# alevar/tiebrush

Hardware: AMD Instinct MI355X
Metric: input alignment records/sec collapsed (tiebrush) + bases/sec covered (tiecov) (higher is better)
Workload: dtype int64; 1 GPU; c3: 64 synthetic sorted BAMs x 5000000 100bp reads per GPU, --clip collapse + tiecov -c -j of the result; records_per_gpu=320000000, groups_out=25086541, parallelism=files-per-rank x1, ranks_seen=1, resident=SoA in HBM before the timed region, contexts=3

## Files before the change

### tiebrush_amd/csrc/tbk_api.hip

```cpp
#include <sys/mman.h>

#include <algorithm>
#include <chrono>
#include <mutex>
#include <vector>
#include <new>

#include "tbk_internal.h"

namespace {
std::mutex g_reg_m;
struct RegEntry {
  void* p;
  int users;
};
std::vector<RegEntry> g_reg;
}

static void release_registered(tbk_ctx* ctx) {
  if (ctx->registered.empty()) return;
  (void)hipStreamSynchronize(ctx->stream);
  const auto r0 = std::chrono::steady_clock::now();
  struct RP {
    tbk_ctx* c;
// ... 369 lines not shown
  return ctx->aux;
}

tbk_ctx* tbk_side_ctx(tbk_ctx* ctx) {
  if (!ctx->side_ctx && tbk_create(ctx->device, &ctx->side_ctx) != 0) ctx->side_ctx = nullptr;
  if (ctx->side_ctx) {
    ctx->side_ctx->profiling = ctx->profiling;
    ctx->side_ctx->dbg = ctx->dbg;
  }
  return ctx->side_ctx;
}
int tbk_side_begin(tbk_ctx* side, size_t arena_hint) {
  if (hipSetDevice(side->device) != hipSuccess) return TBK_EHIP;
  tbk_prof_begin_call(side);
  return ws_begin_call(side, arena_hint);
}
void tbk_side_end(tbk_ctx* side) { tbk_prof_end_call(side); }

static void merge_side_times(tbk_ctx* ctx) {
  if (!ctx->side_times_pending || !ctx->side_ctx) return;
  ctx->side_times_pending = false;
  for (auto& t : ctx->side_ctx->last_times) {
    bool found = false;
    for (auto& u : ctx->last_times)
      if (strcmp(u.name, t.name) == 0) {
        u.ms += t.ms;
        u.launches += t.launches;
        found = true;
        break;
      }
    if (!found) ctx->last_times.push_back(t);
  }
}

static int yd_stage_on(tbk_ctx* run_on, void* job, size_t hint) {
  if (hipSetDevice(run_on->device) != hipSuccess) return TBK_EHIP;
  tbk_prof_begin_call(run_on);
  int rc = ws_begin_call(run_on, hint);
  if (rc == 0) rc = tbk_collapse_yd_run(run_on, job);
  tbk_prof_end_call(run_on);
  return rc;
}

static int finish_yd(tbk_ctx* ctx) {
  if (!ctx->yd_pending) return 0;
  ctx->yd_worker->wait();
  ctx->yd_pending = false;
  ctx->ws_base_off = 0;
  if (ctx->yd_ctx) {
    ctx->last_times = ctx->yd_ctx->last_times;
    if (ctx->yd_rc != 0) ctx->last_error = ctx->yd_ctx->last_error;
  }
  return ctx->yd_rc;
}

void tbk_debug_parse(const char* spec, TbkDebug* out) {
  *out = TbkDebug();
  if (!spec) return;
  std::string s(spec);
  size_t at = 0;
  while (at < s.size()) {
    size_t end = s.find(',', at);
    if (end == std::string::npos) end = s.size();
    const std::string kv = s.substr(at, end - at);
    at = end + 1;
    const size_t eq = kv.find('=');
    const std::string k = kv.substr(0, eq), v = eq == std::string::npos ? std::string("1") : kv.substr(eq + 1);
    const unsigned long long u = strtoull(v.c_str(), nullptr, 0);
    const bool on = v != "0";
    if (k == "path") out->path = v == "sort" ? 1 : (v == "window" ? 2 : 0);
    else if (k == "raw") out->raw = on ? 1 : 0;
    else if (k == "sort") out->sort = v == "radix" ? 1 : (v == "runs" ? 2 : 0);
    else if (k == "scan") out->scan = v == "lookback" ? 1 : (v == "3pass" ? 2 : 0);
    else if (k == "hash_mask") out->hash_mask = (uint32_t)u;
    else if (k == "qhash_mask") out->qhash_mask = u;
    else if (k == "yd_wave_min") out->yd_wave_min = (uint32_t)u;
    else if (k == "yd_bgrid") out->yd_bgrid = (uint32_t)u;
    else if (k == "yd_radix") out->yd_radix = on;
    else if (k == "yd_literal") out->yd_literal = on;
    else if (k == "yd_front") out->yd_front_split = v == "split";
    else if (k == "yd_own_arena") out->yd_own_arena = on;
    else if (k == "wg_stats") out->wg_stats = on;
    else if (k == "wg_og") out->wg_og = (uint32_t)u;
    else if (k == "wg_dense_verify") out->wg_dense_verify = on;
    else if (k == "wg_rank_merge") out->wg_rank_merge = on;
    else if (k == "wg_back") out->wg_back_split = v == "split";
    else if (k == "cov_legacy") out->cov_legacy = on;
    else if (k == "cov_bundle_scan") out->cov_bundle_scan = on;
    else if (k == "cov_prep") out->cov_prep = on;
    else if (k == "cov_tile_cap") out->cov_tile_cap = u;
    else if (k == "junc_radix") out->junc_radix = on;
    else if (k == "no_junc_agg") out->no_junc_agg = on;
    else if (k == "jh_cap") out->jh_cap = (uint32_t)u;
    else if (k == "index_chain") out->index_chain = on;
    else if (k == "no_register") out->no_register = on;
    else if (k == "phases") out->phases = on;
    else if (k == "no_bounce") out->no_bounce = on;
    else if (k == "fmt_slice") out->fmt_slice = u;
  }
}

extern "C" {

int tbk_abi_version(void) { return TBK_ABI_VERSION; }

int tbk_set_debug(tbk_ctx* ctx, const char* spec) {
  if (!ctx) return TBK_EINVAL;
  tbk_debug_parse(spec, &ctx->dbg);
  if (ctx->yd_ctx) ctx->yd_ctx->dbg = ctx->dbg;
  if (ctx->side_ctx) ctx->side_ctx->dbg = ctx->dbg;
  return 0;
}

const char* tbk_strerror(int s) {
  switch (s) {
    case TBK_OK: return "ok";
    case TBK_EINVAL: return "invalid argument";
    case TBK_ENOMEM: return "out of memory";
    case TBK_EHIP: return "HIP runtime error";
    case TBK_E2BIG: return "output capacity too small";
    case TBK_EUNSUPPORTED: return "option or input outside the supported/pinned semantics";
    case TBK_EUNSORTED: return "input not coordinate-sorted";
    case TBK_EFATALOP: return "unknown opcode (tiecov accepts only M/I/D/N/S)";
    case TBK_ECOLLISION: return "key hash collision survived all reseeds";
    case TBK_ENODEVICE: return "no usable gfx950 device";
  }
  return "unknown status";
}

int tbk_create(int device_ordinal, tbk_ctx** out) {
  if (!out) return TBK_EINVAL;
  *out = nullptr;
  int ndev = 0;
  if (hipGetDeviceCount(&ndev) != hipSuccess || ndev <= 0 || device_ordinal < 0 || device_ordinal >= ndev) return TBK_ENODEVICE;
  tbk_ctx* ctx = new (std::nothrow) tbk_ctx();
  if (!ctx) return TBK_ENOMEM;
  ctx->device = device_ordinal;
  tbk_debug_parse(getenv("TBK_DEBUG"), &ctx->dbg);
  bool ok = hipSetDevice(device_ordinal) == hipSuccess;
  hipDeviceProp_t prop;
  if (ok && hipGetDeviceProperties(&prop, device_ordinal) == hipSuccess) ctx->num_cu = prop.multiProcessorCount;
  ok = ok && hipStreamCreateWithFlags(&ctx->own_stream, hipStreamNonBlocking) == hipSuccess;
  ctx->stream = ctx->own_stream;
  ok = ok && hipMalloc((void**)&ctx->d_scalars, 64 * sizeof(uint64_t)) == hipSuccess;
  if (ok) ctx->d_err = (uint32_t*)(ctx->d_scalars + 15);
  ok = ok && hipHostMalloc((void**)&ctx->h_scalars, (64 + 4096) * sizeof(uint64_t), hipHostMallocDefault) == hipSuccess;
  if (!ok) {
    tbk_destroy(ctx);
    return TBK_EHIP;
  }
  *out = ctx;
  return 0;
}

int tbk_collapse_finish_yd(tbk_ctx* ctx) {
  if (!ctx) return TBK_EINVAL;
  return finish_yd(ctx);
}

void tbk_destroy(tbk_ctx* ctx) {
  if (!ctx) return;
  (void)finish_yd(ctx);
  tbk_bam_release(ctx);
  delete ctx->yd_worker;
  ctx->yd_worker = nullptr;
  delete ctx->side_worker;
// ... 449 lines not shown
```

### tiebrush_amd/csrc/tbk_internal.h

```cpp
#pragma once
#include <hip/hip_runtime.h>
#include <stdint.h>
#include <stdio.h>
#include <string.h>

#include <string>
#include <condition_variable>
#include <functional>
#include <mutex>
#include <thread>
#include <utility>
#include <vector>

#include "../../include/tbk.h"

enum : uint32_t {
  TBK_DERR_UNSORTED = 1u << 0,
  TBK_DERR_COLLISION = 1u << 1,
  TBK_DERR_FATALOP = 1u << 2,
  TBK_DERR_SPAN = 1u << 3,
  TBK_DERR_NCIGAR = 1u << 4,
  TBK_DERR_FRACTIONAL = 1u << 5,
  TBK_DERR_OVERFLOW = 1u << 6,
  TBK_DERR_INTERNAL = 1u << 7,
  TBK_DERR_BIGBUCKET = 1u << 8,
  TBK_DERR_RAWORDER = 1u << 9
};

struct KTime {
  const char* name;
  hipEvent_t a, b;
};

struct TbkWorker {
  std::thread th;
  std::mutex m;
  std::condition_variable cv;
  std::function<void()> job;
  bool busy = false, quit = false, started = false;
  void post(std::function<void()> j) {
    {
      std::lock_guard<std::mutex> lk(m);
      if (!started) {
        started = true;
        th = std::thread([this]() {
          std::unique_lock<std::mutex> lk2(m);
          for (;;) {
            cv.wait(lk2, [&] { return quit || (bool)job; });
            if (quit) return;
            std::function<void()> run = std::move(job);
            job = nullptr;
            lk2.unlock();
            run();
            lk2.lock();
            busy = false;
            cv.notify_all();
          }
        });
      }
      job = std::move(j);
      busy = true;
    }
    cv.notify_all();
  }
  void wait() {
    std::unique_lock<std::mutex> lk(m);
    cv.wait(lk, [&] { return !busy; });
  }
  ~TbkWorker() {
    {
      std::lock_guard<std::mutex> lk(m);
      quit = true;
    }
    cv.notify_all();
    if (th.joinable()) th.join();
  }
};

struct TbkDebug {
  int path = 0;
  int raw = -1;
  int sort = 0;
  int scan = 0;
  uint32_t hash_mask = 0xFFFFFFFFu;
  uint64_t qhash_mask = ~0ull;
  uint32_t yd_wave_min = 0;
  uint32_t yd_bgrid = 0;
  bool yd_radix = false;
  bool yd_literal = false;
  bool yd_front_split = false;
  bool yd_own_arena = false;
  uint32_t wg_og = 0;
  bool wg_stats = false;
  bool wg_dense_verify = false, wg_rank_merge = false;
  bool wg_back_split = false;
  bool cov_legacy = false, cov_bundle_scan = false, cov_prep = false, junc_radix = false, no_junc_agg = false;
  uint64_t cov_tile_cap = 0;
  uint32_t jh_cap = 0;
  bool index_chain = false;
  bool no_register = false;
  bool no_bounce = false;
  bool phases = false;
  uint64_t fmt_slice = 0;
};
void tbk_debug_parse(const char* spec, TbkDebug* out);

struct tbk_ctx {
  int device = 0;
  TbkDebug dbg;
  hipStream_t own_stream = nullptr;
  hipStream_t stream = nullptr;
  hipStream_t aux = nullptr;
  hipEvent_t aux_done = nullptr;
  char* ws = nullptr;
  size_t ws_cap = 0, ws_off = 0;
  size_t ws_top = 0;
  bool ws_top_mode = false;
  bool ws_borrowed = false;
  std::vector<std::pair<char*, size_t>> ws_overflow;
  size_t ws_over_used = 0;
  uint32_t* d_err = nullptr;
  uint64_t* d_scalars = nullptr;
  uint64_t* h_scalars = nullptr;
  hipEvent_t stage_ev = nullptr;
  char* d_view = nullptr;
  size_t d_view_cap = 0;
  struct ViewPrep {
    bool valid = false;
    const void* cig = nullptr;
    uint32_t n = 0;
    int32_t *start = nullptr, *end = nullptr, *yi = nullptr;
    uint32_t *jcnt = nullptr, *ridx = nullptr;
    const void* agg = nullptr;
    uint32_t agg_tiles = 0;
    uint64_t n_bases = 0, sum_abs = 0, n_junc = 0;
    uint32_t err = 0;
  } view_prep;
  bool profiling = false;
  std::vector<KTime> ktimes;
  std::vector<hipEvent_t> ev_pool;
  size_t ev_used = 0;
  std::vector<tbk_kernel_time> last_times;
  std::string last_error;
  tbk_collapse_route route{};
  int num_cu = 256;
  void* yd_job = nullptr;
  tbk_ctx* yd_ctx = nullptr;
  TbkWorker* yd_worker = nullptr;
  bool yd_pending = false;
  int yd_rc = 0;
  size_t ws_base_off = 0;
  tbk_ctx* side_ctx = nullptr;
  TbkWorker* side_worker = nullptr;
  bool side_times_pending = false;
  std::vector<void*> registered;
  char* d_unpack = nullptr;
  size_t d_unpack_cap = 0;
  std::vector<uint8_t> unpack_tbm;
  void* bam_dev = nullptr;
  void* enc = nullptr;
  void* ix = nullptr;
  void* stager = nullptr;
  char* bounce = nullptr;
  char* kept = nullptr;
  size_t kept_cap = 0;
  uint32_t kept_n = 0;
  uint32_t* kept_rep = nullptr;
  double* kept_yc = nullptr;
  int64_t* kept_yx = nullptr;
  int32_t* kept_yd = nullptr;
  char* d_names = nullptr;
  uint64_t* d_name_off = nullptr;
  uint32_t n_names = 0;
  void* fmt_pin[2] = {nullptr, nullptr};
  size_t fmt_pin_cap = 0;
// ... 107 lines not shown
```

### tiebrush_amd/csrc/wgroup.h

```cpp
#pragma once
#include <stdlib.h>

#include "strategy.hpp"
#include "tbk_internal.h"

struct WgOut {
  uint32_t ng = 0, np = 0;
  uint64_t *ghi = nullptr, *glo = nullptr;
  uint32_t* gmem = nullptr;
  uint32_t* gpoff = nullptr;
  uint16_t* pfile = nullptr;
  uint32_t* pgrp = nullptr;
  uint64_t* gfmask = nullptr;
  uint32_t* rec_sg = nullptr;
  double* yc = nullptr;
  uint32_t* ns = nullptr;
  long long *yxin = nullptr, *ydin = nullptr;
  unsigned long long* rep = nullptr;
  uint32_t* first = nullptr;
  uint8_t* tie = nullptr;
  uint32_t *gperm = nullptr, *ginv = nullptr;
  bool ties_done = false;
};

struct WgDirectOut {
  uint32_t cap = 0;
  uint32_t* rep = nullptr;
  double* yc = nullptr;
  int64_t* yx = nullptr;
  int32_t *g_start = nullptr, *g_end = nullptr, *rep_effend = nullptr;
  uint64_t* g_key = nullptr;
  int strategy = 0;
};

int tbk_window_groups(tbk_ctx* ctx, const tbkd::ColIn& I, int strategy, const uint64_t* chi, const uint64_t* clo, const uint32_t* cval,
                      const uint32_t* ceff, uint32_t m, const uint32_t* d_run_off, uint64_t* scratch_hi, uint64_t* scratch_lo,
                      bool want_rec_sg, uint64_t seed, WgOut* out, uint32_t* err_bits, const tbkd::ColOpt* raw_opt = nullptr, bool part = false,
                      const WgDirectOut* direct = nullptr );
bool tbk_window_supported(uint32_t k);
inline bool tbk_yd_by_list(const tbk_ctx* ctx, uint32_t k) { return 2u * k <= 128u && !ctx->dbg.yd_radix; }

int tbk_partial_reduce_device(tbk_ctx* ctx, int strategy, const int32_t* rows, uint32_t n2, const uint32_t* run_off_host, uint32_t n_runs,
                              const uint32_t* cig, tbk_groups_out* out, tbk_cov_in* view, const uint32_t* md_off = nullptr,
                              const uint8_t* md = nullptr, const uint8_t* md_has = nullptr);
```

### tiebrush_amd/csrc/wgroup.hip

```cpp
#include <stdlib.h>

#include <algorithm>

#include "dev_common.hpp"
#include "strategy.hpp"
#include "tbk_internal.h"
#include "wgroup.h"

namespace {

constexpr int WG_NT = 512;
constexpr int WG_E = 8;
constexpr int WG_CAP = WG_NT * WG_E;
constexpr uint32_t WG_T = 1024;
constexpr uint32_t WG_KS = 2048;
constexpr int WG_NW = WG_NT / 64;
constexpr int WG_R = 4;
constexpr int WG_RS = 1;
constexpr int WG_RR = 1;

__global__ void wg_sample_k(const uint64_t* __restrict__ chi, uint32_t m, uint32_t s, uint32_t ns, uint64_t* __restrict__ shi) {
  uint32_t j = blockIdx.x * blockDim.x + threadIdx.x;
  if (j >= ns) return;
  uint64_t d = (uint64_t)j * s;
// ... 158 lines not shown
      }
    } else {
      for (uint32_t j = t; j < i1 - i0; j += 256) key[j] = chi[i0 + j] >> 2;
    }
    __syncthreads();
    uint32_t f_first;
    {
      uint32_t lo = 0, hi = k;
      while (hi - lo > 1) {
        const uint32_t mid = (lo + hi) >> 1;
        if (s_run[mid] <= i0)
          lo = mid;
        else
          hi = mid;
      }
      f_first = lo;
    }
    uint32_t seg = 0;
    for (uint32_t f = f_first; f < k; ++f) {
      const uint32_t a = s_run[f], b = s_run[f + 1];
      if (a >= i1) break;
      if (b <= i0 || a == b) continue;
      const uint32_t sa = a > i0 ? a : i0, sb = b < i1 ? b : i1;
      const bool has_lo = sa > a;
      const bool cont = has_lo && c_f == f && c_end == sa;
      const uint64_t klo = !has_lo ? 0ull : cont ? c_klast : (RAW ? raw_key(rtid[sa - 1], rpos[sa - 1]) : (chi[sa - 1] >> 2));
      const uint64_t khi = key[sb - 1 - i0];
      uint32_t r_lo, r_hi;
      bool found = false, have_v = false;
      if (cont && sb == b) {
        r_lo = c_rhi;
        r_hi = nW;
        found = true;
      } else if (cont) {
        r_lo = c_rhi;
        const bool le = r_lo + t < nW && wprobe <= khi;
        const uint64_t mb = __ballot(le);
        uint32_t* sl = s_loc[(g + seg) & 1u];
        if ((t & 63u) == 0) sl[t >> 6] = (uint32_t)__builtin_popcountll(mb);
        __syncthreads();
        const uint32_t c = sl[0] + sl[1] + sl[2] + sl[3];
        if (c < 256u) {
          r_hi = r_lo + c;
          found = true;
          have_v = true;
        }
      }
      ++seg;
      if (!found) {
        upper_bounds2(klo, !has_lo, khi, sb == b, &r_lo, &r_hi);
        r_hi = sb == b ? nW : r_hi;
      }
      const uint64_t v_mine = wprobe;
      if (sb != b) {
        c_f = f;
        c_end = sb;
        c_rhi = r_hi;
        c_klast = khi;
        wprobe = r_hi + t < nW ? W[r_hi + t] : ~0ull;
      } else {
        c_f = ~0u;
      }
      for (uint32_t r = r_lo + t; r < r_hi; r += 256) {
        const uint64_t v = have_v ? v_mine : W[r];
        uint32_t lo = sa - i0, hi = sb - i0;
        while (lo < hi) {
          const uint32_t mid = lo + ((hi - lo) >> 1);
          if (key[mid] < v)
            lo = mid + 1;
          else
            hi = mid;
        }
        offT[(size_t)f * nrows + (r + 1)] = i0 + lo;
      }
      if (RAW) {
        for (uint32_t j = sa + t; j < sb; j += 256) {
          const uint64_t pk = j > sa ? key[j - 1 - i0] : klo;
          bad |= pk > key[j - i0];
        }
      }
    }
  }
  if (RAW && bad) atomicOr(err, TBK_DERR_RAWORDER);
}
__global__ void wg_offsets_edges_k(const uint32_t* __restrict__ run_off, uint32_t k, uint32_t nrows, uint32_t* __restrict__ offT) {
  const uint32_t f = blockIdx.x;
  const uint32_t a = run_off[f], b = run_off[f + 1];
  uint32_t* col = offT + (size_t)f * nrows;
  if (threadIdx.x == 0) {
    col[0] = a;
    col[nrows - 1] = b;
  }
  if (a == b)
    for (uint32_t r = 1 + threadIdx.x; r + 1 < nrows; r += blockDim.x) col[r] = a;
}
__global__ __launch_bounds__(256) void wg_offsets_transpose_k(const uint32_t* __restrict__ offT, uint32_t k, uint32_t nrows, uint32_t* __restrict__ off,
                                                             uint32_t* __restrict__ wbase) {
  __shared__ uint32_t tile[64][65];
  const uint32_t r0 = blockIdx.x * 64, f0 = blockIdx.y * 64;
  const uint32_t tx = threadIdx.x & 63, ty = threadIdx.x >> 6;
  const uint32_t start = (wbase && tx < k) ? offT[(size_t)tx * nrows] : 0u;
  for (uint32_t y = ty; y < 64; y += 4) {
    const uint32_t f = f0 + y, r = r0 + tx;
    if (f < k && r < nrows) tile[y][tx] = offT[(size_t)f * nrows + r];
  }
  __syncthreads();
  for (uint32_t y = ty; y < 64; y += 4) {
    const uint32_t r = r0 + y, f = f0 + tx;
    const bool in = f < k && r < nrows;
    const uint32_t v = in ? tile[tx][y] : 0u;
    if (in) off[(size_t)r * k + f] = v;
    if (wbase) {
      const uint32_t sum = wave_sum(in ? v - start : 0u);
      if (tx == 0 && r < nrows) wbase[r] = sum;
    }
  }
}
struct WgRaw {
  ColIn I;
  ColOpt O;
  unsigned long long* n_pass;
  unsigned long long* n_slots;
  uint32_t all_slots;
  uint32_t sparse;
};
constexpr uint32_t WG_NSPREAD = 64, WG_SPREAD_STRIDE = 16;
__device__ __forceinline__ void wg_count(unsigned long long* base, unsigned long long v) {
  atomicAdd(base + (size_t)(blockIdx.x & (WG_NSPREAD - 1u)) * WG_SPREAD_STRIDE, v);
}
__device__ __forceinline__ uint32_t wave_seg_max(uint32_t x, uint32_t f, uint32_t* fo) {
#define WG_SEG_STEP(ctrl, rm)                                                                  \
  {                                                                                            \
    const uint32_t xo = (uint32_t)__builtin_amdgcn_update_dpp(0, (int)x, ctrl, rm, 0xf, false); \
    const uint32_t fq = (uint32_t)__builtin_amdgcn_update_dpp(0, (int)f, ctrl, rm, 0xf, false); \
    x = f ? x : (xo > x ? xo : x);                                                             \
    f |= fq;                                                                                   \
  }
  WG_SEG_STEP(0x111, 0xf)
  WG_SEG_STEP(0x112, 0xf)
  WG_SEG_STEP(0x114, 0xf)
  WG_SEG_STEP(0x118, 0xf)
  WG_SEG_STEP(0x142, 0xa)
  WG_SEG_STEP(0x143, 0xc)
#undef WG_SEG_STEP
  *fo = f;
  return x;
}
struct RawA {
  int32_t pos, tidv, ppos, ptid;
  uint32_t fl_mq_sc;
  int32_t nh;
  uint32_t c0, nc;
};
struct RawRec {
  uint64_t hi, lo, rk, prk;
  uint32_t x;
  uint32_t err;
  bool pass;
};
__device__ __forceinline__ RawA wg_raw_a(const ColIn& I, uint32_t i, bool need_prev) {
  RawA a;
  a.pos = I.pos[i];
  a.tidv = I.tid[i];
  a.fl_mq_sc = (uint32_t)I.flag[i] | ((uint32_t)I.mapq[i] << 16) | (strand_code(I.strand[i]) << 24);
  a.nh = I.nh[i];
  a.c0 = I.cig_off[i];
// ... 1621 lines not shown
      const uint32_t src = rsrc[e];
      const int4* rp = reinterpret_cast<const int4*>(rows + (size_t)src * TBK_PARTIAL_ROW);
      const int4 a = rp[0], b = rp[1], c = rp[2];
      const uint32_t eff = (uint32_t)a.w;
      if (m == q || eff < beff) {
        beff = eff;
        best = src;
      }
      yc += (double)(uint32_t)b.z;
      yx += (uint32_t)b.w;
      yd = (uint32_t)c.x > yd && c.x > 0 ? (uint32_t)c.x : yd;
      if (hashed && m > q && !strategy_equal(I, strategy, src, rsrc[e0])) atomicOr(err, TBK_DERR_COLLISION);
    }
    T.rep[wb + gid] = best;
    T.yc[wb + gid] = yc;
    if (yx > 0xFFFFFFFFull) atomicOr(err, TBK_DERR_OVERFLOW);
    T.yx[wb + gid] = (uint32_t)yx;
    T.yd[wb + gid] = yd;
    T.khi[wb + gid] = h;
    T.klo[wb + gid] = l;
    ++gid;
  }
  if (t == 0) T.wg_cnt[w] = tot;
}

__global__ __launch_bounds__(256) void pr_compact_k(uint32_t nw, const uint32_t* __restrict__ wbase, PrTemp T, const uint32_t* __restrict__ gbase,
                                                   uint32_t cap, uint32_t* __restrict__ o_rep,
                                                   double* __restrict__ o_yc, int64_t* __restrict__ o_yx, int32_t* __restrict__ o_yd,
                                                   int32_t* __restrict__ o_start, int32_t* __restrict__ o_end, uint64_t* __restrict__ o_key,
                                                   int strategy) {
  const uint32_t w = blockIdx.x * 4u + (threadIdx.x >> 6);
  if (w >= nw) return;
  const uint32_t ng = T.wg_cnt[w];
  if (!ng) return;
  const uint32_t wb = wbase[w], gb = gbase[w];
  for (uint32_t g = threadIdx.x & 63u; g < ng; g += 64) {
    const uint32_t o = gb + g;
    if (o >= cap) continue;
    const uint32_t r = T.rep[wb + g], yxv = T.yx[wb + g], ydv = T.yd[wb + g];
    const double ycv = T.yc[wb + g];
    const uint64_t h = T.khi[wb + g], l = T.klo[wb + g];
    o_rep[o] = r;
    o_yc[o] = ycv;
    o_yx[o] = (int64_t)yxv;
    o_yd[o] = (int32_t)ydv;
    if (o_start || o_end || o_key) {
      const int32_t start = (int32_t)((h >> 2) & 0x7FFFFFFFull);
      if (o_start) o_start[o] = start;
      if (o_end) o_end[o] = start + (int32_t)(uint32_t)(l >> 32) - 1;
      if (o_key) {
        const uint32_t word = (uint32_t)l;
        uint32_t shape = 0;
        if (strategy == TBK_STRAT_CIGAR || strategy == TBK_STRAT_CLIP) {
          if (word == (0x80000000u | C_M)) shape = 0x80000000u;
          if ((word >> 30) == 3u) shape = word;
        }
        o_key[2 * (size_t)o] = h;
        o_key[2 * (size_t)o + 1] = (l & 0xFFFFFFFF00000000ull) | shape;
      }
    }
  }
}

__global__ __launch_bounds__(64) void wg_spread_sum_k(const unsigned long long* __restrict__ spread, unsigned long long* __restrict__ n_pass,
                                                      unsigned long long* __restrict__ n_slots) {
  const unsigned long long a = wave_sum(spread[(size_t)threadIdx.x * WG_SPREAD_STRIDE]);
  const unsigned long long b = wave_sum(spread[(size_t)(WG_NSPREAD + threadIdx.x) * WG_SPREAD_STRIDE]);
  if (threadIdx.x == 0) {
    *n_pass += a;
    *n_slots += b;
  }
}

}

bool tbk_window_supported(uint32_t k) { return k >= 1 && k <= 1024; }

static int wg_offsets_build(tbk_ctx* ctx, bool raw, const uint64_t* chi, const int32_t* rtid, const int32_t* rpos, const int32_t* ctid,
                            const uint32_t* d_run_off, uint32_t k,
                            uint32_t m, const uint64_t* W, uint32_t nW, uint32_t nrows, uint32_t* off, uint32_t* wbase ) {
  uint32_t* offT = ws_alloc<uint32_t>(ctx, (size_t)nrows * k);
  if (!offT) return TBK_ENOMEM;
  const uint32_t og = std::min<uint32_t>(WG_OG, std::max<uint32_t>(1u, ctx->dbg.wg_og ? ctx->dbg.wg_og : m / (WG_OC * 2048u)));
  if (raw)
    TBK_LAUNCH(ctx, "wg_offsets", wg_offsets_stream_k<true>, cdiv(m, WG_OC * og), 256, 0, chi, rtid, rpos, ctid, d_run_off, k, m, W, nW, nrows, offT, ctx->d_err, og);
  else
    TBK_LAUNCH(ctx, "wg_offsets", wg_offsets_stream_k<false>, cdiv(m, WG_OC * og), 256, 0, chi, rtid, rpos, ctid, d_run_off, k, m, W, nW, nrows, offT, ctx->d_err, og);
  TBK_LAUNCH(ctx, "wg_offsets_edges", wg_offsets_edges_k, k, 256, 0, d_run_off, k, nrows, offT);
  TBK_LAUNCH(ctx, "wg_offsets_transpose", wg_offsets_transpose_k, dim3(cdiv(nrows, 64u), cdiv(k, 64u)), 256, 0, offT, k, nrows, off,
             k <= 64 ? wbase : nullptr);
  if (k > 64) TBK_LAUNCH(ctx, "wg_rowsum", wg_rowsum_k, cdiv(nrows, 4), 256, 0, off, k, nrows, wbase);
  return 0;
}

int tbk_partial_reduce_device(tbk_ctx* ctx, int strategy, const int32_t* rows, uint32_t n2, const uint32_t* run_off_host, uint32_t k,
                              const uint32_t* cig, tbk_groups_out* out, tbk_cov_in* view, const uint32_t* md_off, const uint8_t* md,
                              const uint8_t* md_has) {
  if (strategy == TBK_STRAT_FULL && !md_off) return TBK_EINVAL;
  if (k > PR_MAXRUNS) return TBK_EUNSUPPORTED;
  const uint32_t B = 256, m = n2;
  uint64_t* sc = ctx->d_scalars;
  TBK_HIP(hipMemsetAsync(sc, 0, 16 * sizeof(uint64_t), ctx->stream));
  uint32_t* d_run_off = ws_alloc<uint32_t>(ctx, (size_t)k + 1);
  if (!d_run_off) return TBK_ENOMEM;
  {
    void* stage = tbk_stage_acquire(ctx);
    memcpy(stage, run_off_host, (size_t)(k + 1) * 4);
    TBK_HIP(hipMemcpyAsync(d_run_off, stage, (size_t)(k + 1) * 4, hipMemcpyHostToDevice, ctx->stream));
    tbk_stage_release(ctx);
  }
  uint64_t* chi = ws_alloc<uint64_t>(ctx, m);
  int32_t* r_tid = ws_alloc<int32_t>(ctx, m);
  int32_t* r_pos = ws_alloc<int32_t>(ctx, m);
  uint8_t* r_strand = ws_alloc<uint8_t>(ctx, m);
  uint32_t* ncig = ws_alloc<uint32_t>(ctx, m);
  uint32_t* cig_off = ws_alloc<uint32_t>(ctx, (size_t)m + 1);
  if (!cig_off) return TBK_ENOMEM;
  TBK_LAUNCH(ctx, "pr_rowkeys", pr_rowkeys_k, cdiv(m, B), B, 0, m, rows, chi, r_tid, r_pos, r_strand, ncig);
  TBK_TRY(tbk_exscan_u32(ctx, ncig, cig_off, m, sc + 23));
  TBK_LAUNCH(ctx, "pr_tail", pr_tail_k, 1, 1, 0, m, sc + 23, cig_off);
  uint32_t s = 1;
  while (s * 2 * k <= PR_KS && s * 2 <= PR_T) s *= 2;
  const uint32_t g = PR_T / s;
  const uint32_t ns = cdiv(m, s);
  const uint32_t nsp = ns > 1 ? (ns - 1) / g : 0;
  const uint32_t nW = 2 * nsp, nw = nW + 1, nrows = nw + 1;
  uint64_t* W = ws_alloc<uint64_t>(ctx, (size_t)nW + 1);
  uint32_t* off = ws_alloc<uint32_t>(ctx, (size_t)nrows * k);
  uint32_t* wbase = ws_alloc<uint32_t>(ctx, (size_t)nw + 1);
  uint32_t* gbase = ws_alloc<uint32_t>(ctx, nw);
  PrTemp T;
  T.rep = ws_alloc<uint32_t>(ctx, m);
  T.yc = ws_alloc<double>(ctx, m);
  T.yx = ws_alloc<uint32_t>(ctx, m);
  T.yd = ws_alloc<uint32_t>(ctx, m);
  T.khi = ws_alloc<uint64_t>(ctx, m);
  T.klo = ws_alloc<uint64_t>(ctx, m);
  T.wg_cnt = ws_alloc<uint32_t>(ctx, nw);
  if (!W || !off || !wbase || !gbase || !T.wg_cnt || !T.klo) return TBK_ENOMEM;
  if (nsp) {
    uint64_t* Z = ws_alloc<uint64_t>(ctx, (size_t)ns / g + 2);
    if (!Z) return TBK_ENOMEM;
    TBK_LAUNCH(ctx, "pr_sample_rank", pr_sample_rank_k, cdiv(ns, B), B, 0, chi, m, s, ns, d_run_off, k, g, Z);
    TBK_LAUNCH(ctx, "wg_split", wg_split_k, cdiv(nsp, B), B, 0, Z, 1u, nsp, W);
  }
  TBK_TRY(wg_offsets_build(ctx, false, chi, nullptr, nullptr, nullptr, d_run_off, k, m, W, nW, nrows, off, wbase));
  ColIn I{};
  I.n = m;
  I.k = k;
  I.pos = r_pos;
  I.cig_off = cig_off;
  I.cig = cig;
  I.md_off = md_off;
  I.md = md;
  I.md_has = md_has;
  TBK_LAUNCH(ctx, "pr_merge", pr_merge_k, nw, PR_NT, 0, rows, off, k, nw, wbase, I, strategy, T, ctx->d_err);
  TBK_TRY(tbk_exscan_u32(ctx, T.wg_cnt, gbase, nw, sc + 1));
  uint32_t eb = 0;
  TBK_TRY(tbk_sync_err(ctx, &eb));
  if (eb & TBK_DERR_BIGBUCKET) {
    ctx->last_error = "more partials start on one base than a workgroup merges";
    return TBK_E2BIG;
  }
  if (eb) return tbk_derr_to_status(ctx, eb);
  const uint32_t ng = (uint32_t)ctx->h_scalars[1];
  out->n_groups = ng;
  if (ng > out->cap_groups) return TBK_E2BIG;
  if (ng == 0) return 0;
  uint64_t* okey = out->g_key;
  if (view && !okey) {
    okey = ws_alloc<uint64_t>(ctx, 2 * (size_t)ng);
    if (!okey) return TBK_ENOMEM;
  }
  TBK_LAUNCH(ctx, "pr_compact", pr_compact_k, cdiv(nw, 4u), 256, 0, nw, wbase, T, gbase, out->cap_groups, out->rep, out->yc, out->yx, out->yd,
             out->g_start, out->g_end, okey, strategy);
// ... 306 lines not shown
```

Baseline: 22.18 billion records/s.

## Add wave-per-chunk raw window offset kernel with LDS-staged keys

Adds a new kernel that computes per-file window offsets with one wavefront per contiguous chunk, staging keys in LDS (32-bit position keys when a chunk has a single tid, 64-bit otherwise) and bisecting window boundaries cooperatively with ballots. It becomes the default for raw input when the tid/pos pointers are 16-byte aligned, replacing the block-level stream kernel, and carries run state across chunks. A debug knob restores the old block path, and a standalone entry point for raw offsets is also added. It aims to cut binary-search and global-load cost in the offsets pass, at the price of more complex control flow and possible per-wave divergence.

```diff
diff --git a/tiebrush_amd/csrc/tbk_api.hip b/tiebrush_amd/csrc/tbk_api.hip
--- a/tiebrush_amd/csrc/tbk_api.hip
+++ b/tiebrush_amd/csrc/tbk_api.hip
@@ -475,6 +475,7 @@
     else if (k == "yd_own_arena") out->yd_own_arena = on;
     else if (k == "wg_stats") out->wg_stats = on;
     else if (k == "wg_og") out->wg_og = (uint32_t)u;
+    else if (k == "wg_offsets") out->wg_offsets_block = v == "block";
     else if (k == "wg_dense_verify") out->wg_dense_verify = on;
     else if (k == "wg_rank_merge") out->wg_rank_merge = on;
     else if (k == "wg_back") out->wg_back_split = v == "split";
diff --git a/tiebrush_amd/csrc/tbk_internal.h b/tiebrush_amd/csrc/tbk_internal.h
--- a/tiebrush_amd/csrc/tbk_internal.h
+++ b/tiebrush_amd/csrc/tbk_internal.h
@@ -91,6 +91,7 @@
   bool yd_front_split = false;
   bool yd_own_arena = false;
   uint32_t wg_og = 0;
+  bool wg_offsets_block = false;
   bool wg_stats = false;
   bool wg_dense_verify = false, wg_rank_merge = false;
   bool wg_back_split = false;
diff --git a/tiebrush_amd/csrc/wgroup.h b/tiebrush_amd/csrc/wgroup.h
--- a/tiebrush_amd/csrc/wgroup.h
+++ b/tiebrush_amd/csrc/wgroup.h
@@ -38,6 +38,8 @@
                       bool want_rec_sg, uint64_t seed, WgOut* out, uint32_t* err_bits, const tbkd::ColOpt* raw_opt = nullptr, bool part = false,
                       const WgDirectOut* direct = nullptr );
 bool tbk_window_supported(uint32_t k);
+int tbk_wg_offsets_raw(tbk_ctx* ctx, const int32_t* tid, const int32_t* pos, const uint32_t* d_run_off, uint32_t k, uint32_t n, const uint64_t* W,
+                       uint32_t nW, uint32_t* off, uint32_t* wbase);
 inline bool tbk_yd_by_list(const tbk_ctx* ctx, uint32_t k) { return 2u * k <= 128u && !ctx->dbg.yd_radix; }
 
 int tbk_partial_reduce_device(tbk_ctx* ctx, int strategy, const int32_t* rows, uint32_t n2, const uint32_t* run_off_host, uint32_t n_runs,
diff --git a/tiebrush_amd/csrc/wgroup.hip b/tiebrush_amd/csrc/wgroup.hip
--- a/tiebrush_amd/csrc/wgroup.hip
+++ b/tiebrush_amd/csrc/wgroup.hip
@@ -264,6 +264,257 @@
     }
   }
   if (RAW && bad) atomicOr(err, TBK_DERR_RAWORDER);
+}
+constexpr uint32_t WV_ST = 1024;
+__device__ __forceinline__ uint32_t wv_upper_bound(const uint64_t* __restrict__ W, uint32_t lo, uint32_t hi, uint64_t v, uint32_t lane) {
+  while (lo < hi) {
+    const uint32_t step = (hi - lo + 63u) >> 6;
+    const uint32_t p = lo + lane * step;
+    const bool le = p < hi && W[p] <= v;
+    const uint32_t T = (uint32_t)__builtin_popcountll(__ballot(le));
+    if (T == 0) {
+      hi = lo;
+    } else {
+      const uint32_t pT = lo + T * step;
+      hi = T < 64u && pT < hi ? pT : hi;
+      lo = lo + (T - 1u) * step + 1u;
+      lo = lo > hi ? hi : lo;
+    }
+  }
+  return lo;
+}
+struct WvPos {
+  using K = uint32_t;
+  static constexpr uint32_t NQ = 4;
+  uint64_t base;
+  __device__ __forceinline__ K of(uint64_t v) const {
+    const uint64_t d = v - base;
+    return v <= base ? 0u : d > 0x7FFFFFFFull ? 0x80000000u : (uint32_t)d;
+  }
+  __device__ __forceinline__ uint64_t full(K x) const { return base | x; }
+};
+struct WvKey {
+  using K = uint64_t;
+  static constexpr uint32_t NQ = 2;
+  __device__ __forceinline__ K of(uint64_t v) const { return v; }
+  __device__ __forceinline__ uint64_t full(K x) const { return x; }
+};
+struct WvState {
+  uint32_t f;
+  bool have_ab;
+  uint32_t a, b;
+  bool carry;
+  uint32_t c_rhi;
+  uint64_t c_klast, wp[3];
+  bool bad;
+};
+template <uint32_t NQ>
+__device__ __forceinline__ void wv_load(const int32_t* __restrict__ src, uint32_t i0, uint32_t n, uint32_t lane, int32_t* v) {
+  const uint32_t rem = n - i0;
+#pragma unroll
+  for (uint32_t q = 0; q < NQ; ++q) {
+    const uint32_t o = 256u * q + 4u * lane;
+    if (o < rem && rem - o >= 4u) {
+      const int4 x = *reinterpret_cast<const int4*>(src + (size_t)i0 + o);
+      v[4 * q] = x.x, v[4 * q + 1] = x.y, v[4 * q + 2] = x.z, v[4 * q + 3] = x.w;
+    } else {
+#pragma unroll
+      for (uint32_t e = 0; e < 4; ++e) v[4 * q + e] = o + e < rem ? src[(size_t)i0 + o + e] : 0;
+    }
+  }
+}
+__device__ __forceinline__ void wv_probes(const uint64_t* __restrict__ W, uint32_t nW, uint32_t r, uint32_t lane, uint64_t (&wp)[3]) {
+#pragma unroll
+  for (uint32_t i = 0; i < 3; ++i) wp[i] = r < nW && nW - r > lane + 64u * i ? W[r + lane + 64u * i] : ~0ull;
+}
+template <uint32_t NC, uint32_t LEN, class K>
+__device__ __forceinline__ void wv_bisect(const K* key, uint32_t lo0, uint32_t hi0, const K (&p)[3], uint32_t (&res)[3]) {
+  uint32_t lo[NC], hi[NC];
+#pragma unroll
+  for (uint32_t c = 0; c < NC; ++c) lo[c] = lo0, hi[c] = hi0;
+  const uint32_t iters = 32u - (uint32_t)__builtin_clz(hi0 - lo0);
+  for (uint32_t it = 0; it < iters; ++it) {
+#pragma unroll
+    for (uint32_t c = 0; c < NC; ++c) {
+      const uint32_t mid = lo[c] + ((hi[c] - lo[c]) >> 1);
+      const bool open = lo[c] < hi[c];
+      const bool lt = key[mid < LEN ? mid : LEN - 1u] < p[c];
+      lo[c] = open && lt ? mid + 1u : lo[c];
+      hi[c] = open && !lt ? mid : hi[c];
+    }
+  }
+#pragma unroll
+  for (uint32_t c = 0; c < NC; ++c) res[c] = lo[c];
+}
+template <class D>
+__device__ __forceinline__ void wv_step(const D dom, typename D::K* key, typename D::K (&kq)[4 * D::NQ], uint32_t i0, uint32_t i1, uint32_t lane,
+                                        const int32_t* __restrict__ rtid, const int32_t* __restrict__ rpos, const int32_t* __restrict__ ctid,
+                                        const uint32_t* __restrict__ run_off, uint32_t k, uint32_t n, const uint64_t* __restrict__ W, uint32_t nW,
+                                        uint32_t nrows, uint32_t* __restrict__ offT, WvState& S) {
+  using K = typename D::K;
+  constexpr uint32_t NQ = D::NQ, LEN = 256u * NQ;
+  const uint32_t len = i1 - i0;
+  __builtin_amdgcn_wave_barrier();
+#pragma unroll
+  for (uint32_t q = 0; q < NQ; ++q) {
+#pragma unroll
+    for (uint32_t e = 0; e < 4; ++e) {
+      const uint32_t j = 256u * q + 4u * lane + e;
+      kq[4 * q + e] = j < len ? kq[4 * q + e] : (K)~(K)0;
+      key[j] = kq[4 * q + e];
+    }
+  }
+  __builtin_amdgcn_fence(__ATOMIC_RELEASE, "wavefront");
+  __builtin_amdgcn_wave_barrier();
+  __builtin_amdgcn_fence(__ATOMIC_ACQUIRE, "wavefront");
+  uint64_t pk0 = 0;
+  uint32_t nocmp = 0;
+  while (S.f < k) {
+    if (!S.have_ab) {
+      S.a = run_off[S.f];
+      S.b = run_off[S.f + 1];
+      S.have_ab = true;
+    }
+    const uint32_t f = S.f, a = S.a, b = S.b;
+    if (a >= i1) break;
+    if (b <= i0 || a == b || b > n || a > b) {
+      ++S.f;
+      S.have_ab = false;
+      continue;
+    }
+    const uint32_t sa = a > i0 ? a : i0, sb = b < i1 ? b : i1;
+    const bool has_lo = sa > a;
+    const bool cont = has_lo && S.carry;
+    uint64_t klo = 0;
+    if (cont) {
+      klo = S.c_klast;
+    } else if (has_lo) {
+      const int32_t pc = ctid[(sa - 1u) / WG_TC];
+      klo = raw_key(pc != WG_TC_MIXED ? pc : rtid[sa - 1u], rpos[sa - 1u]);
+    }
+    if (has_lo) {
+      pk0 = klo;
+    } else if (sa > i0) {
+      const uint32_t j = sa - i0;
+      nocmp |= lane == ((j & 255u) >> 2) ? 1u << ((j >> 8) * 4u + (j & 3u)) : 0u;
+    }
+    const uint64_t khi = dom.full(key[sb - 1u - i0]);
+    const bool ends = sb == b;
+    uint32_t r = cont ? S.c_rhi : has_lo ? wv_upper_bound(W, 0u, nW, klo, lane) : 0u;
+    uint64_t wp[3];
+    if (cont) {
+#pragma unroll
+      for (uint32_t i = 0; i < 3; ++i) wp[i] = S.wp[i];
+    } else {
+      wv_probes(W, nW, r, lane, wp);
+    }
+    uint32_t* const col = offT + (size_t)f * nrows + 1u;
+    for (;;) {
+      const K pd[3] = {dom.of(wp[0]), dom.of(wp[1]), dom.of(wp[2])};
+      uint32_t res[3];
+      const bool t0 = r < nW && lane < nW - r && (ends || wp[0] <= khi);
+      const uint32_t c0 = (uint32_t)__builtin_popcountll(__ballot(t0));
+      uint32_t tot = c0;
+      if (c0 < 64u) {
+        wv_bisect<1, LEN, K>(key, sa - i0, sb - i0, pd, res);
+        if (t0) col[r + lane] = i0 + res[0];
+      } else {
+        const bool t1 = lane + 64u < nW - r && (ends || wp[1] <= khi);
+        const uint32_t c1 = (uint32_t)__builtin_popcountll(__ballot(t1));
+        const bool t2 = c1 == 64u && lane + 128u < nW - r && (ends || wp[2] <= khi);
+        const uint32_t c2 = (uint32_t)__builtin_popcountll(__ballot(t2));
+        tot = 64u + c1 + c2;
+        wv_bisect<3, LEN, K>(key, sa - i0, sb - i0, pd, res);
+        col[r + lane] = i0 + res[0];
+        if (t1) col[r + lane + 64u] = i0 + res[1];
+        if (t2) col[r + lane + 128u] = i0 + res[2];
+      }
+      r += tot;
+      if (tot < 192u) break;
+      wv_probes(W, nW, r, lane, wp);
+    }
+    if (!ends) {
+      S.carry = true;
+      S.c_rhi = r;
+      S.c_klast = khi;
+      wv_probes(W, nW, r, lane, S.wp);
+      break;
+    }
+    S.carry = false;
+    ++S.f;
+    S.have_ab = false;
+  }
+  const K pk0d = dom.of(pk0);
+  bool bad = false;
+#pragma unroll
+  for (uint32_t q = 0; q < NQ; ++q) {
+    const uint32_t j0 = 256u * q + 4u * lane;
+    K x[4];
+#pragma unroll
+    for (uint32_t e = 0; e < 4; ++e) x[e] = key[j0 + e];
+    const K prev = key[j0 ? j0 - 1u : 0u];
+    const K before = j0 ? prev : pk0d;
+#pragma unroll
+    for (uint32_t e = 0; e < 4; ++e) {
+      const K pk = e == 0 ? before : x[e - 1];
+      bad |= pk > x[e] && !((nocmp >> (4 * q + e)) & 1u);
+    }
+  }
+  S.bad |= bad;
+}
+__global__ __launch_bounds__(256) void wg_offsets_wave_k(const int32_t* __restrict__ rtid, const int32_t* __restrict__ rpos,
+                                                         const int32_t* __restrict__ ctid, const uint32_t* __restrict__ run_off, uint32_t k,
+                                                         uint32_t n, const uint64_t* __restrict__ W, uint32_t nW, uint32_t nrows,
+                                                         uint32_t* __restrict__ offT, uint32_t* __restrict__ err, uint32_t steps ) {
+  __shared__ __attribute__((aligned(16))) uint32_t s_key[4][WV_ST];
+  const uint32_t lane = threadIdx.x & 63u;
+  const uint32_t wid = (uint32_t)__builtin_amdgcn_readfirstlane((int)(threadIdx.x >> 6));
+  const uint64_t start64 = (uint64_t)(blockIdx.x * 4u + wid) * steps * WV_ST;
+  if (start64 >= n) return;
+  const uint32_t start = (uint32_t)start64;
+  const uint32_t end = n - start < steps * WV_ST ? n : start + steps * WV_ST;
+  WvState S;
+  {
+    uint32_t lo = 0, hi = k;
+    while (hi - lo > 1) {
+      const uint32_t mid = (lo + hi) >> 1;
+      if (run_off[mid] <= start)
+        lo = mid;
+      else
+        hi = mid;
+    }
+    S.f = lo;
+  }
+  S.have_ab = false;
+  S.a = S.b = 0;
+  S.carry = false;
+  S.c_rhi = 0;
+  S.c_klast = 0;
+  S.wp[0] = S.wp[1] = S.wp[2] = ~0ull;
+  S.bad = false;
+  for (uint32_t i0 = start; i0 < end;) {
+    int32_t npos[16];
+    wv_load<4>(rpos, i0, n, lane, npos);
+    const int32_t ct = ctid[i0 / WG_TC];
+    uint32_t i1;
+    if (ct != WG_TC_MIXED) {
+      i1 = end - i0 < WV_ST ? end : i0 + WV_ST;
+      uint32_t kq[16];
+#pragma unroll
+      for (uint32_t u = 0; u < 16; ++u) kq[u] = ct < 0 ? 0u : (uint32_t)npos[u] & 0x7FFFFFFFu;
+      wv_step(WvPos{raw_key(ct, 0)}, &s_key[wid][0], kq, i0, i1, lane, rtid, rpos, ctid, run_off, k, n, W, nW, nrows, offT, S);
+    } else {
+      i1 = end - i0 < WV_ST / 2u ? end : i0 + WV_ST / 2u;
+      int32_t nt[8];
+      wv_load<2>(rtid, i0, n, lane, nt);
+      uint64_t kq[8];
+#pragma unroll
+      for (uint32_t u = 0; u < 8; ++u) kq[u] = raw_key(nt[u], npos[u]);
+      wv_step(WvKey{}, reinterpret_cast<uint64_t*>(&s_key[wid][0]), kq, i0, i1, lane, rtid, rpos, ctid, run_off, k, n, W, nW, nrows, offT, S);
+    }
+    i0 = i1;
+  }
+  if (S.bad) atomicOr(err, TBK_DERR_RAWORDER);
 }
 __global__ void wg_offsets_edges_k(const uint32_t* __restrict__ run_off, uint32_t k, uint32_t nrows, uint32_t* __restrict__ offT) {
   const uint32_t f = blockIdx.x;
@@ -2051,7 +2302,12 @@
   uint32_t* offT = ws_alloc<uint32_t>(ctx, (size_t)nrows * k);
   if (!offT) return TBK_ENOMEM;
   const uint32_t og = std::min<uint32_t>(WG_OG, std::max<uint32_t>(1u, ctx->dbg.wg_og ? ctx->dbg.wg_og : m / (WG_OC * 2048u)));
-  if (raw)
+  const bool wave = raw && !ctx->dbg.wg_offsets_block && (((uintptr_t)rtid | (uintptr_t)rpos) & 15u) == 0;
+  if (wave) {
+    const uint32_t steps = og * (WG_OC / WV_ST);
+    TBK_LAUNCH(ctx, "wg_offsets", wg_offsets_wave_k, cdiv(cdiv(m, WV_ST * steps), 4u), 256, 0, rtid, rpos, ctid, d_run_off, k, m, W, nW, nrows, offT, ctx->d_err,
+               steps);
+  } else if (raw)
     TBK_LAUNCH(ctx, "wg_offsets", wg_offsets_stream_k<true>, cdiv(m, WG_OC * og), 256, 0, chi, rtid, rpos, ctid, d_run_off, k, m, W, nW, nrows, offT, ctx->d_err, og);
   else
     TBK_LAUNCH(ctx, "wg_offsets", wg_offsets_stream_k<false>, cdiv(m, WG_OC * og), 256, 0, chi, rtid, rpos, ctid, d_run_off, k, m, W, nW, nrows, offT, ctx->d_err, og);
@@ -2060,6 +2316,16 @@
              k <= 64 ? wbase : nullptr);
   if (k > 64) TBK_LAUNCH(ctx, "wg_rowsum", wg_rowsum_k, cdiv(nrows, 4), 256, 0, off, k, nrows, wbase);
   return 0;
+}
+
+int tbk_wg_offsets_raw(tbk_ctx* ctx, const int32_t* tid, const int32_t* pos, const uint32_t* d_run_off, uint32_t k, uint32_t n, const uint64_t* W,
+                       uint32_t nW, uint32_t* off, uint32_t* wbase) {
+  if (!tbk_window_supported(k) || n == 0) return TBK_EINVAL;
+  const uint32_t nchunks = cdiv(n, WG_TC);
+  int32_t* ctid = ws_alloc<int32_t>(ctx, nchunks);
+  if (!ctid) return TBK_ENOMEM;
+  TBK_LAUNCH(ctx, "wg_sample", wg_tidchunks_k, cdiv(nchunks, 256u), 256, 0, tid, n, d_run_off, k, nchunks, ctid);
+  return wg_offsets_build(ctx, true, nullptr, tid, pos, ctid, d_run_off, k, n, W, nW, nW + 2u, off, wbase);
 }
 
 int tbk_partial_reduce_device(tbk_ctx* ctx, int strategy, const int32_t* rows, uint32_t n2, const uint32_t* run_off_host, uint32_t k,
```

Measured after the change: 22.58 billion records/s, median of 6. +1.8%, better.
